# ohseokkwon/Foveated-Rendering-using-Ray-Tracing

Measured on AMD Instinct MI355X. Metric: Mrays/s + reconstructed fps @4K, 10% foveal density, 1/2/4/8 GPU, higher is better.
Workload: dtype f32

## Files before the change

foveated-rendering-using-ray-tracing_amd/csrc/ctx_buffers.cpp:

```cpp
#include <algorithm>
#include <array>

#include "ctx_internal.h"

using namespace fr;
using namespace fri;

namespace {
constexpr uint32_t kSnapMagic = 0x4E535246u;
constexpr uint32_t kSnapVersion = 1;
struct SnapHeader {
  uint32_t magic, version;
  int32_t width, height, pp_S, spp, scene, mask_mode;
  uint32_t accum, light_pending;
  float light_emission[3];
  int32_t diffuse_max_depth;
  float inv_vp[16], prev_vp[16], eye[3], prev_eye[3], gaze[2];
  uint64_t payload_bytes;
};
struct SnapPart {
  void* dev;
  size_t bytes;
};
std::array<SnapPart, 7> snap_parts(fr_ctx* c) {
// ... 168 lines not shown
  c->extra.settle(c);
  join_recon(c);
  hipSetDevice(c->cfg.device);
  const char* in = static_cast<const char*>(host);
  size_t off = sizeof(h);
  for (const SnapPart& p : snap_parts(c)) {
    HIP_TRY(c, hipMemcpyAsync(p.dev, in + off, p.bytes, hipMemcpyHostToDevice, c->stream));
    off += p.bytes;
  }
  HIP_TRY(c, hipStreamSynchronize(c->stream));
  c->accum = h.accum;
  c->light_pending = h.light_pending != 0;
  c->dsc.light_emission = mk3(h.light_emission[0], h.light_emission[1], h.light_emission[2]);
  c->U.diffuse_max_depth = h.diffuse_max_depth;
  c->U.mask_mode = h.mask_mode;
  memcpy(&c->U.inv_vp, h.inv_vp, sizeof(h.inv_vp));
  memcpy(&c->U.prev_vp, h.prev_vp, sizeof(h.prev_vp));
  memcpy(&c->U.eye, h.eye, sizeof(h.eye));
  memcpy(&c->U.prev_eye, h.prev_eye, sizeof(h.prev_eye));
  memcpy(&c->U.gaze, h.gaze, sizeof(h.gaze));
  c->lp_gaze = f2{-1e30f, -1e30f};
  c->lp_mode = -1;
  c->sib_prefix_fresh = false;
  c->hvalid_fresh = false;
  c->moved = false;
  return FR_OK;
}

}
```

foveated-rendering-using-ray-tracing_amd/csrc/ctx_create.cpp:

```cpp
#include <cmath>
#include <cstdlib>

#include "ctx_internal.h"

using namespace fr;
using fri::fail;

static thread_local std::string g_create_error;

int fri::fail(fr_ctx* c, int code, const std::string& msg) {
  if (c) c->err = msg; else g_create_error = msg;
  return code;
}

extern "C" {

const char* fr_version(void) { return "fovrt 0.2 (gfx950)"; }
int fr_abi_version(void) { return FOVRT_ABI_VERSION; }

int fr_config_default(fr_config* c) {
  if (!c) return FR_E_INVALID;
  memset(c, 0, sizeof(*c));
  c->abi_version = FOVRT_ABI_VERSION;
  c->width = 1024; c->height = 1024;
// ... 48 lines not shown
      return FR_TEX_F32;
    }
    out[i] = word;
  }
  return FR_TEX_RGBE;
}

static void read_env_knobs(fr_ctx* c) {
  if (const char* v = getenv("FOVRT_SHADE_CHUNK_REFR")) c->chunk_refr = (uint32_t)std::max(0, atoi(v));
  if (const char* v = getenv("FOVRT_SHADE_XCD_BANDS")) c->xcd_bands = atoi(v) != 0;
  if (const char* v = getenv("FOVRT_SHADE_HANDOFF")) c->handoff = (uint32_t)std::min(std::max(atoi(v), 0), 2);
  if (const char* v = getenv("FOVRT_TEX_PACKING")) c->tex_packing = atoi(v) != 0;
  if (const char* v = getenv("FOVRT_JFA_LAZY_OUTPUTS")) c->lazy_jfa_outputs = atoi(v) != 0;
  if (const char* v = getenv("FOVRT_EARLY_SETUP")) c->early_setup = atoi(v) != 0;
  if (const char* v = getenv("FOVRT_EXTRA_LAZY")) c->extra_lazy = atoi(v) != 0;
  if (const char* v = getenv("FOVRT_SIB_STRIP")) c->sib_strip = atoi(v) != 0;
  if (const char* v = getenv("FOVRT_SLOTS")) c->nslots = std::max(2, std::min(fr_ctx::MAX_SLOTS, atoi(v)));
  {
    const char* v = getenv("FOVRT_SHADE_BLOCKS_PER_CU");
    const int full = fr::shade_max_blocks_per_cu();
    c->shade_blocks_per_cu = v ? std::max(1, std::min(full, atoi(v))) : full;
  }
  if (const char* v = getenv("FOVRT_JFA_XCD")) c->jfa_xcd = atoi(v);
  if (const char* v = getenv("FOVRT_SIB_STRIP_MID")) c->sib_strip_mid = atoi(v);
  if (const char* v = getenv("FOVRT_ATROUS_ROWS2")) c->atrous_rows2 = atoi(v) != 0;
  if (const char* v = getenv("FOVRT_ATROUS_XCD")) c->atrous_xcd = atoi(v) != 0;
}

static std::vector<hipEvent_t*> timed_events(fr_ctx* c) {
  fr_ctx::StageEvents& t = c->tev;
  std::vector<hipEvent_t*> v = {&t.begin, &t.geometry, &t.sampling, &t.optimize, &t.shading, &t.end, &t.paths_begin,
                                &t.paths_end, &t.chain2_begin, &t.pullpush, &t.atrous, &t.chain1_begin, &t.jfa,
                                &t.sibson, &t.stage_begin, &t.stage_end, &c->ev_carry_fork, &c->ev_carry_done,
                                &c->ev_recon_fork, &c->ev_chain2_done, &c->ev_stream_join};
  for (auto& s : c->lat.ev)
    for (hipEvent_t* e : {&s.front_begin, &s.front_end, &s.jfa_end, &s.recon_end}) v.push_back(e);
  return v;
}

int fr_create(const fr_config* cfg_in, fr_ctx** out) {
  if (!out) return fail(nullptr, FR_E_INVALID, "out is NULL");
  *out = nullptr;
  fr_config cfg;
  if (cfg_in) cfg = *cfg_in; else fr_config_default(&cfg);
  if (cfg.abi_version != FOVRT_ABI_VERSION)
    return fail(nullptr, FR_E_INVALID, "fr_config.abi_version != FOVRT_ABI_VERSION (initialise it with fr_config_default)");
// ... 167 lines not shown
  const size_t atlas = (size_t)c->pp_S * (c->pp_S + c->pp_S / 2);
  if (compaction_tiles(c->W, c->H) > 1024) { c->err = "screen too large for the compaction scan"; return bail(FR_E_UNSUPPORTED); }
  for (int k = 0; k < c->nslots; k++)
    if (dalloc(&c->mask_p[k], N) != hipSuccess || dalloc(&c->ray_count_p[k], 4) != hipSuccess ||
        dalloc(&c->active_p[k], N) != hipSuccess) {
      c->err = "device allocation (work buffers) failed";
      return bail(FR_E_NOMEM);
    }
  c->mask = c->mask_p[0]; c->ray_count = c->ray_count_p[0]; c->active = c->active_p[0];
  for (int k = 0; k < fr_ctx::MAX_SLOTS; k++)
    if (dalloc(&c->owner_counts_p[k], FR_MAX_SHARD_RANKS) != hipSuccess) {
      c->err = "device allocation (work buffers) failed";
      return bail(FR_E_NOMEM);
    }
  if (dalloc(&c->bcount, nblocks) != hipSuccess ||
      hipHostMalloc((void**)&c->h_counts, sizeof(uint32_t) * fr_ctx::MAX_SLOTS * FR_MAX_SHARD_RANKS) != hipSuccess) {
    c->err = "allocation (shard counts) failed";
    return bail(FR_E_NOMEM);
  }
  memset(c->h_counts, 0, sizeof(uint32_t) * fr_ctx::MAX_SLOTS * FR_MAX_SHARD_RANKS);
  if (dalloc(&c->gclass, N) != hipSuccess || dalloc(&c->lp_cache, N) != hipSuccess ||
      dalloc(&c->lp_inv, logpolar_inv_words(c->W, c->H)) != hipSuccess || dalloc(&c->words, nwords) != hipSuccess ||
      dalloc(&c->counts, 4 * nblocks) != hipSuccess || dalloc(&c->offsets, 4 * nblocks) != hipSuccess ||
      dalloc(&c->tiles, 1024) != hipSuccess || dalloc(&c->jfa_a, N) != hipSuccess || dalloc(&c->jfa_b, N) != hipSuccess ||
      dalloc(&c->pull, atlas) != hipSuccess || dalloc(&c->push, atlas) != hipSuccess ||
      dalloc(&c->snap, pp_snap_count(c->pp_S)) != hipSuccess || dalloc(&c->stats, 1) != hipSuccess ||
      dalloc(&c->shade_ctr, shade_counter_words()) != hipSuccess || dalloc(&c->samples, std::max(N * cfg.spp, 2 * shade_fx_slots((uint32_t)N, cfg.spp, c->handoff, c->shade_blocks_per_cu))) != hipSuccess ||
      dalloc(&c->sample_help, std::max<size_t>(4 * shade_fx_slots((uint32_t)N, cfg.spp, c->handoff, c->shade_blocks_per_cu), 1)) != hipSuccess ||
      dalloc(&c->aux_p[0], N) != hipSuccess || dalloc(&c->aux_seed_p[0], N) != hipSuccess ||
      dalloc(&c->aux_p[1], N) != hipSuccess || dalloc(&c->aux_seed_p[1], N) != hipSuccess ||
      dalloc(&c->hvalid, N / 64 + 1) != hipSuccess ||
      hipMalloc((void**)&c->item_store, shade_item_store_f4(c->shade_blocks_per_cu) * sizeof(f4)) != hipSuccess ||
      (cfg.sibson_mode == 0 && (dalloc(&c->sib_prefix, (size_t)(c->W + 1) * c->H) != hipSuccess ||
                                dalloc(&c->sib_blocks, (size_t)sibson_prefix_blocks(c->W) * c->H) != hipSuccess ||
                                hipMalloc((void**)&c->sib_wide, ((size_t)c->W * c->H + 2) * sizeof(uint32_t)) != hipSuccess ||
                                hipMalloc((void**)&c->sib_strips, sibson_strip_words(c->W, c->H) * sizeof(uint32_t)) != hipSuccess ||
                                dalloc(&c->sib_rowp, sibson_rowp_texels(c->W, c->H)) != hipSuccess))) {
    c->err = "device allocation (work buffers) failed";
    return bail(FR_E_NOMEM);
  }
  c->aux = c->aux_p[0];
  c->aux_seed = c->aux_seed_p[0];
  {
    std::vector<float> ft((size_t)c->W + c->H);
    for (int x = 0; x < c->W; x++) ft[x] = ((float)x + 0.5f) / (float)c->W;
    for (int y = 0; y < c->H; y++) ft[(size_t)c->W + y] = ((float)y + 0.5f) / (float)c->H;
    if (!up(&c->ftab, ft)) { c->err = "device allocation (work buffers) failed"; return bail(FR_E_NOMEM); }
// ... 34 lines not shown
  const hipStream_t streams[5] = {c->stream, c->atrous_stream, c->sibson_stream, c->carry_stream, c->front_stream};
  for (hipStream_t s : streams) if (s) hipStreamSynchronize(s);
  auto fr = [](void* p) { if (p) hipFree(p); };
  fr(c->d_nodes); fr(c->d_tri); fr(c->d_prim); fr(c->d_shade); fr(c->d_pos);
  fr(c->spare_nodes); fr(c->spare_tri); fr(c->spare_prim); fr(c->spare_pos); fr(c->prev_pos); fr(c->shade_back);
  fr(c->pose_rest_pos); fr(c->pose_rest_nrm); fr(c->pose_stage_pos); fr(c->pose_stage_nrm);
  if (c->bvh_work) bvh_work_free(c->bvh_work);
  if (c->sah_work) sah_work_free(c->sah_work);
  if (c->nrm_work) normals_work_free(c->nrm_work);
  for (auto p : c->d_tex) fr(p);
  fr(c->d_mats); fr(c->d_texs);
  for (auto p : c->img) fr(p);
  for (int k = 0; k < fr_ctx::MAX_SLOTS; k++) { fr(c->mask_p[k]); fr(c->ray_count_p[k]); fr(c->active_p[k]); fr(c->owner_counts_p[k]); }
  fr(c->bcount); fr(c->shard_map); fr(c->front_need); fr(c->shade_radiance);
  if (c->h_counts) hipHostFree(c->h_counts);
  fr(c->geo);
  if (c->h_geo) hipHostFree(c->h_geo);
  fr(c->rb);
  if (c->h_rb) hipHostFree(c->h_rb);
  if (c->geo_read.ev) hipEventDestroy(c->geo_read.ev);
  for (auto& f : c->set_read) if (f.ev) hipEventDestroy(f.ev);
  if (c->update_done.ev) hipEventDestroy(c->update_done.ev);
  for (auto e : c->ev_counts) if (e) hipEventDestroy(e);
  fr(c->gclass); fr(c->lp_cache); fr(c->lp_inv); fr(c->words); fr(c->counts); fr(c->offsets); fr(c->tiles); fr(c->shade_ctr); fr(c->samples); fr(c->sample_help); fr(c->aux_p[0]); fr(c->aux_p[1]); fr(c->aux_seed_p[0]); fr(c->aux_seed_p[1]); fr(c->hvalid); fr(c->item_store); fr(c->jfa_a); fr(c->jfa_b); fr(c->ftab);
  fr(c->pull); fr(c->push); fr(c->snap); fr(c->stats); fr(c->sib_prefix); fr(c->sib_blocks); fr(c->sib_wide); fr(c->sib_strips); fr(c->sib_rowp);
  for (hipEvent_t* e : timed_events(c)) if (*e) hipEventDestroy(*e);
  if (c->front_done.ev) hipEventDestroy(c->front_done.ev);
  for (auto& f : c->trace_done) if (f.ev) hipEventDestroy(f.ev);
  for (auto& f : c->recon_done) if (f.ev) hipEventDestroy(f.ev);
  for (auto& f : c->jfa_done) if (f.ev) hipEventDestroy(f.ev);
  for (auto& q : c->kt_ev)
    for (auto e : q) if (e) hipEventDestroy(e);
  for (auto& q : c->fc_ev)
    for (auto e : q) if (e) hipEventDestroy(e);
  if (c->fc_ref) hipEventDestroy(c->fc_ref);
  for (hipStream_t s : streams) if (s) hipStreamDestroy(s);
  delete c;
  return FR_OK;
}

int fr_set_camera(fr_ctx* c, const fr_camera* cam) {
  if (!c || !cam) return FR_E_INVALID;
  FrameUniforms& U = c->U;
  memcpy(U.inv_vp.m, cam->inv_vp, sizeof(U.inv_vp.m));
  memcpy(U.prev_vp.m, cam->prev_vp, sizeof(U.prev_vp.m));
  U.eye = mk3(cam->eye[0], cam->eye[1], cam->eye[2]);
  U.prev_eye = mk3(cam->prev_eye[0], cam->prev_eye[1], cam->prev_eye[2]);
// ... 44 lines not shown
```

foveated-rendering-using-ray-tracing_amd/csrc/ctx_frame.cpp:

```cpp
#include <immintrin.h>
#include <sched.h>

#include <chrono>
#include <cmath>
#include <functional>

#include "ctx_internal.h"

using namespace fr;
using namespace fri;

namespace {
constexpr float kPollDeadlineMs = 10000.0f;
inline void cpu_relax() { _mm_pause(); }
hipError_t poll_event(hipEvent_t ev, float deadline_ms) {
  const auto t0 = std::chrono::steady_clock::now();
  for (uint32_t n = 1;; n++) {
    const hipError_t e = hipEventQuery(ev);
    if (e != hipErrorNotReady) return e;
    if ((n & 63u) == 0) {
      if (std::chrono::duration<float, std::milli>(std::chrono::steady_clock::now() - t0).count() > deadline_ms)
        return hipErrorNotReady;
      sched_yield();
    } else {
// ... 219 lines not shown
    case FR_BUF_DEPTH_CACHE: *phys = c->depth_cache; return FR_OK;
    case FR_BUF_DIFFUSE: *phys = P_DIFFUSE; return FR_OK;
    case FR_BUF_WEIGHT: *phys = P_wgt(c); return FR_OK;
    case FR_BUF_HISTORY: *phys = c->hist_cur; return FR_OK;
    case FR_BUF_HISTORY_CACHE: *phys = c->hist_cache; return FR_OK;
    case FR_BUF_SHADING: *phys = P_shd(c); return FR_OK;
    case FR_BUF_EXTRA: *phys = P_EXTRA; return FR_OK;
    case FR_BUF_JFA_COORD: *phys = P_JFA_COORD; return FR_OK;
    case FR_BUF_JFA_COLOR: *phys = P_JFA_COLOR; return FR_OK;
    case FR_BUF_SIBSON: *phys = P_SIBSON; return FR_OK;
    case FR_BUF_PULLPUSH: *phys = P_PULLPUSH; return FR_OK;
    case FR_BUF_ATROUS: *phys = c->atrous_out; return FR_OK;
    case FR_BUF_LOGPOLAR: *phys = P_LOGPOLAR; return FR_OK;
    case FR_BUF_LOGPOLAR_INVERSE: *phys = P_LOGPOLAR_INV; return FR_OK;
    default: return FR_E_INVALID;
  }
}

static int enqueue_jfa(fr_ctx* c, int in_buffer, hipStream_t stream = nullptr) {
  int p;
  if (resolve(c, in_buffer, &p)) return fail(c, FR_E_INVALID, "jfa: bad input buffer");
  const bool run_form = c->cfg.sibson_mode == 0;
  const bool lazy = run_form && c->lazy_jfa_outputs;
  c->jfa_final = launch_jfa(c->img[p], c->jfa_a, c->jfa_b, c->img[P_JFA_COORD], c->img[P_JFA_COLOR], c->ftab, c->W,
                            c->H, run_form ? c->sib_prefix : nullptr, run_form ? c->sib_blocks : nullptr, !lazy,
                            c->jfa_xcd, stream ? stream : c->stream);
  c->jfa_coord_owed = lazy;
  c->sib_prefix_fresh = run_form;
  return check_launch(c);
}
static int enqueue_sibson(fr_ctx* c, hipStream_t stream = nullptr) {
  if (c->cfg.sibson_mode == 1) {
    materialize_jfa(c, stream ? stream : c->stream);
    launch_sibson(c->img[P_JFA_COORD], c->img[P_JFA_COLOR], c->img[P_SIBSON], c->W, c->H, stream ? stream : c->stream);
  } else {
    launch_sibson_runs(c->img[P_JFA_COORD], c->jfa_final, c->img[P_JFA_COLOR], c->sib_prefix, c->sib_blocks, c->sib_rowp, c->sib_wide,
                       c->sib_strips, c->img[P_SIBSON], c->W, c->H, c->sib_prefix_fresh, c->sib_strip, c->sib_strip_mid,
                       c->jfa_coord_owed,
                       stream ? stream : c->stream);
  }
  return check_launch(c);
}
static int enqueue_pullpush(fr_ctx* c, int in_buffer, hipStream_t stream = nullptr) {
  int p;
  if (resolve(c, in_buffer, &p)) return fail(c, FR_E_INVALID, "pullpush: bad input buffer");
  launch_pullpush(c->img[p], c->pull, c->push, c->snap, c->img[P_PULLPUSH], c->W, c->H, stream ? stream : c->stream);
  return check_launch(c);
}
static int enqueue_atrous(fr_ctx* c, int count, int pos, int nrm, int col, hipStream_t stream = nullptr) {
  if (!stream) stream = c->stream;
  int pp, pn, pc;
  if (count < 1 || resolve(c, pos, &pp) || resolve(c, nrm, &pn) || resolve(c, col, &pc))
// ... 272 lines not shown
```

foveated-rendering-using-ray-tracing_amd/csrc/ctx_internal.h:

```cpp
#pragma once
#include <hip/hip_runtime.h>

#include <cstring>
#include <string>
#include <vector>

#include "../../include/fovrt.h"
#include "fr_device.h"
#include "k_launch.h"
#include "scene.h"

#define FR_MAX_SHARD_RANKS 64

using fr::f2;
using fr::f3;
using fr::u2;
using fr::f4;
using fr::BvhNode;
using fr::TriGeo;
using fr::TriShade;
using fr::DevMaterial;
using fr::DevTexture;
using fr::DevScene;
using fr::DevStats;
// ... 136 lines not shown
  uint8_t* lp_cache = nullptr;
  uint32_t* lp_inv = nullptr;
  f2 lp_gaze{-1e30f, -1e30f};
  int lp_mode = -1;
  unsigned long long* words = nullptr;
  uint32_t* counts = nullptr;
  uint32_t* offsets = nullptr;
  uint32_t* tiles = nullptr;
  uint32_t* ray_count = nullptr;
  uint32_t* active = nullptr;
  uint32_t* shade_ctr = nullptr;
  f4* samples = nullptr;
  unsigned long long* sample_help = nullptr;
  f4* item_store = nullptr;
  f4* aux = nullptr;
  uint32_t* aux_seed = nullptr;
  f4* aux_p[2] = {};
  uint32_t* aux_seed_p[2] = {};
  int aux_i = 0;
  unsigned long long* hvalid = nullptr;
  bool hvalid_fresh = false;
  bool setup_early = false;
  bool early_setup = true;
  u2 *jfa_a = nullptr, *jfa_b = nullptr;
  uint32_t chunk_refr = 0;
  uint32_t xcd_bands = 1;
  uint32_t handoff = 1;
  int shade_blocks_per_cu = 0;
  int jfa_xcd = 1;
  int sib_strip_mid = 0;
  bool atrous_rows2 = true;
  int atrous_xcd = 1;
  float* ftab = nullptr;
  f4 *pull = nullptr, *push = nullptr, *snap = nullptr;
  f4 *sib_prefix = nullptr, *sib_blocks = nullptr;
  uint32_t* sib_wide = nullptr;
  uint32_t* sib_strips = nullptr;
  f4* sib_rowp = nullptr;
  bool sib_prefix_fresh = false;
  const u2* jfa_final = nullptr;
  bool jfa_coord_owed = false;
  bool lazy_jfa_outputs = true;
  struct ExtraDebt {
    bool owed = false;
    FrameUniforms U;
    DevScene sc;
    const float* box = nullptr;
// ... 61 lines not shown
```

foveated-rendering-using-ray-tracing_amd/csrc/ctx_stats.cpp:

```cpp
#include <algorithm>
#include <cstdio>

#include "ctx_internal.h"

using namespace fr;
using namespace fri;

extern "C" {

int fr_get_stats(fr_ctx* c, fr_stats* s) {
  if (!c || !s) return FR_E_INVALID;
  DevStats d;
  HIP_TRY(c, hipMemcpyAsync(&d, c->stats, sizeof(d), hipMemcpyDeviceToHost, c->stream));
  HIP_TRY(c, hipStreamSynchronize(c->stream));
  s->gbuffer_primary = d.gbuffer_primary; s->primary = d.primary; s->shadow = d.shadow;
  s->diffuse_bounce = d.diffuse_bounce; s->mirror = d.mirror; s->refraction = d.refraction;
  s->reflection = d.reflection; s->truncated = d.truncated; s->overflow = d.bvh_overflow;
  for (int i = 0; i < 6; i++) s->diag[i] = d.pad[i];
  s->segments = d.gbuffer_primary + d.primary + d.shadow + d.diffuse_bounce + d.mirror + d.refraction + d.reflection;
  return FR_OK;
}

float fr__sqrt_le_bound(float s) { return sqrt_le_bound(s); }

int fr__sibson_counts(fr_ctx* c, uint32_t* out3) {
  if (!c || !out3 || !c->sib_strips) return FR_E_INVALID;
  hipSetDevice(c->cfg.device);
  HIP_TRY(c, hipDeviceSynchronize());
  HIP_TRY(c, hipMemcpy(out3, c->sib_strips, sizeof(uint32_t), hipMemcpyDeviceToHost));
  HIP_TRY(c, hipMemcpy(out3 + 1, c->sib_wide, 2 * sizeof(uint32_t), hipMemcpyDeviceToHost));
  return FR_OK;
}

int fr_kernel_timing(fr_ctx* c, int enable) {
  if (!c) return FR_E_INVALID;
  if (enable && !c->kt_ev[0][0])
    for (auto& q : c->kt_ev)
      for (auto& e : q) HIP_TRY(c, hipEventCreate(&e));
  c->kt_on = enable != 0;
  c->kt_next = c->kt_pending = 0;
  c->kt_frames = 0;
  c->kt_stage_ms = c->kt_kernel_ms = 0.0;
// ... 141 lines not shown
```

foveated-rendering-using-ray-tracing_amd/csrc/k_jfa.hip:

```cpp
#include <hip/hip_runtime.h>
#include <cmath>
#include "fr_device.h"
#include "k_launch.h"
#include "k_image.h"

namespace fr {


__global__ void k_jfa_init(const f4* __restrict__ in, u2* __restrict__ state, int W, int H, f2 screen) {
  const uint32_t N = (uint32_t)W * (uint32_t)H;
  for (uint32_t p = blockIdx.x * blockDim.x + threadIdx.x; p < N; p += gridDim.x * blockDim.x) {
    const float a = in[p].w;
    const uint32_t y = p / (uint32_t)W;
    const f2 uv = frag_uv(p - y * (uint32_t)W, y, screen);
    state[p] = a >= 1.0f ? u2{__float_as_uint(uv.x) | JFA_FLAG, __float_as_uint(uv.y) | JFA_FLAG}
                         : u2{JFA_UNSEEDED, __float_as_uint(uv.y)};
  }
}


typedef float jfa_v2 __attribute__((ext_vector_type(2)));
FR_DEV u2 jfa_pick(const u2 (&nb)[9], f2 me) {
  float d2[9];
  float dmin = INFINITY;
  const jfa_v2 m = {me.x, me.y};
#pragma unroll
  for (int i = 0; i < 9; i++) {
    const jfa_v2 c = {__uint_as_float(nb[i].x), __uint_as_float(nb[i].y)};
    const jfa_v2 dd = c + m;
    const jfa_v2 sq = dd * dd;
    d2[i] = sq.x + sq.y;
    dmin = fminf(dmin, d2[i]);
  }
  u2 r = nb[0];
  if (dmin != INFINITY) {
    const float bound = sqrt_le_bound(sqrtf(dmin));
#pragma unroll
    for (int i = 8; i >= 0; i--)
      if (d2[i] <= bound) r = nb[i];
// ... 18 lines not shown
  u2 r = nb[0];
  if (dmin != INFINITY) {
    const float bound = sqrt_le_bound(sqrtf(dmin));
    if (down) {
      if (d2[8] <= bound) r = nb[8];
      if (d2[7] <= bound) r = nb[7];
      if (d2[6] <= bound) r = nb[6];
    }
    if (d2[5] <= bound) r = nb[5];
    if (d2[4] <= bound) r = nb[4];
    if (up) {
      if (d2[3] <= bound) r = nb[3];
      if (d2[2] <= bound) r = nb[2];
      if (d2[1] <= bound) r = nb[1];
    }
    if (d2[0] <= bound) r = nb[0];
  }
  return r;
}


template <int JFA_ROWS>
__global__ __launch_bounds__(256) void k_jfa_step(const u2* __restrict__ src, u2* __restrict__ dst, int W, int H,
                                                  int step, const float* __restrict__ ftab, int xcd) {
  const uint32_t t = xcd ? xcd_tile(blockIdx.x, blockIdx.y, gridDim.x, gridDim.y) : blockIdx.y * gridDim.x + blockIdx.x;
  const int x = (int)(t % gridDim.x) * 64 + (threadIdx.x & 63);
  const int g = __builtin_amdgcn_readfirstlane((int)(t / gridDim.x) * 4 + (threadIdx.x >> 6));
  const int base = (g / step) * (JFA_ROWS * step) + g % step;
  if (x >= W || base >= H) return;
  const bool inl = x - step >= 0, inr = x + step < W;
  const int xl = inl ? x - step : x, xr = inr ? x + step : x;
  u2 L[JFA_ROWS + 2], C[JFA_ROWS + 2], R[JFA_ROWS + 2];
  bool in[JFA_ROWS + 2];
  const char* sb = reinterpret_cast<const char*>(src);
  auto ld = [&](uint32_t e) { return *reinterpret_cast<const u2*>(sb + e * 8u); };
#pragma unroll
  for (int m = 0; m < JFA_ROWS + 2; m++) {
    const int yr = base + (m - 1) * step;
    in[m] = yr >= 0 && yr < H;
    if (JFA_ROWS < 4 && !in[m]) {
      L[m] = C[m] = R[m] = u2{JFA_UNSEEDED, 0u};
      continue;
    }
    const uint32_t row = (uint32_t)(in[m] ? yr : base) * (uint32_t)W;
    L[m] = ld(row + (uint32_t)xl);
    C[m] = ld(row + (uint32_t)x);
    R[m] = ld(row + (uint32_t)xr);
    L[m].x = in[m] && inl ? L[m].x : JFA_UNSEEDED;
    C[m].x = in[m] ? C[m].x : JFA_UNSEEDED;
    R[m].x = in[m] && inr ? R[m].x : JFA_UNSEEDED;
  }
#pragma unroll
  for (int k = 0; k < JFA_ROWS; k++) {
    const int y = base + k * step;
    if (y < H) {
      const u2 nb[9] = {C[k + 1], L[k], C[k], R[k], L[k + 1], R[k + 1], L[k + 2], C[k + 2], R[k + 2]};
      *reinterpret_cast<u2*>(reinterpret_cast<char*>(dst) + ((uint32_t)y * (uint32_t)W + (uint32_t)x) * 8u) =
          JFA_ROWS < 4 ? jfa_pick_rows(nb, mk2(ftab[x], ftab[W + y]), in[k], in[k + 2])
                       : jfa_pick(nb, mk2(ftab[x], ftab[W + y]));
    }
  }
}

int jfa_rows(int H, int step) { return std::min(4, (H + step - 1) / step); }
int jfa_row_groups(int H, int step) {
  const int band = jfa_rows(H, step) * step;
  return ((H + band - 1) / band) * step;
}

__global__ void k_jfa_final(const u2* __restrict__ state, const f4* __restrict__ in, f4* __restrict__ coord,
                            f4* __restrict__ color, int W, int H, f2 screen) {
  const size_t N = (size_t)W * H;
  for (size_t p = blockIdx.x * (size_t)blockDim.x + threadIdx.x; p < N; p += (size_t)gridDim.x * blockDim.x) {
    const u2 s = state[p];
    const float sx = jfa_seeded(s.x) ? jfa_coord(s.x) : ((float)(p % (size_t)W) + 0.5f) / screen.x;
    const float sy = jfa_coord(s.y);
    const uint32_t ix = min((uint32_t)floorf(sx * screen.x), (uint32_t)W - 1);
    const uint32_t iy = min((uint32_t)floorf(sy * screen.y), (uint32_t)H - 1);
    const f4 c = in[(size_t)iy * W + ix];
    coord[p] = mk4(sx, sy, 0.0f, c.w);
    color[p] = c;
  }
}

template <bool OUT>
__global__ __launch_bounds__(64) void k_jfa_final_prefix(const u2* __restrict__ state, const f4* __restrict__ in,
                                                         f4* __restrict__ coord, f4* __restrict__ color,
                                                         f4* __restrict__ P, f4* __restrict__ T, int W, int H, int NB,
                                                         f2 screen) {
  const int lane = threadIdx.x;
  const int j = blockIdx.y, B = blockIdx.x;
  const int col = B * 64 + lane;
  f3 v = mk3(0.0f);
  if (col < W) {
    const size_t p = (size_t)j * W + col;
    const u2 s = state[p];
    const float sx = jfa_seeded(s.x) ? jfa_coord(s.x) : ((float)col + 0.5f) / screen.x;
    const float sy = jfa_coord(s.y);
    const uint32_t ix = min((uint32_t)floorf(sx * screen.x), (uint32_t)W - 1);
    const uint32_t iy = min((uint32_t)floorf(sy * screen.y), (uint32_t)H - 1);
    const f4 c = in[(size_t)iy * W + ix];
    if (OUT) coord[p] = mk4(sx, sy, 0.0f, c.w);
    color[p] = c;
    v = xyz(c);
  }
  f3 incl = v;
#pragma unroll
  for (int o = 1; o < 64; o <<= 1) {
    const float tx = __shfl_up(incl.x, o, 64), ty = __shfl_up(incl.y, o, 64), tz = __shfl_up(incl.z, o, 64);
    if (lane >= o) incl = incl + mk3(tx, ty, tz);
  }
  if (col <= W) P[(size_t)j * (W + 1) + col] = mk4(incl - v, 0.0f);
  if (lane == 63) T[(size_t)j * NB + B] = mk4(incl, 0.0f);
}

int jfa_max_step(int W, int H) {
  int m = 1;
  while (m * 2 < W || m * 2 < H) m *= 2;
  return m;
}

const u2* launch_jfa(const f4* in, u2* stateA, u2* stateB, f4* coord, f4* color, const float* ftab, int W, int H,
                     f4* sibP, f4* sibT, bool outputs, int xcd, hipStream_t stream) {
  const size_t N = (size_t)W * H;
  int blocks = (int)std::min<size_t>((N + 255) / 256, 8192);
  f2 screen = mk2((float)W, (float)H);
  hipLaunchKernelGGL(k_jfa_init, dim3(blocks), dim3(256), 0, stream, in, stateA, W, H, screen);
  u2* a = stateA;
  u2* b = stateB;
  for (int step = jfa_max_step(W, H); step >= 1; step /= 2) {
    dim3 grid((W + 63) / 64, (jfa_row_groups(H, step) + 3) / 4);
    auto k = jfa_rows(H, step) == 4 ? k_jfa_step<4> : jfa_rows(H, step) == 3 ? k_jfa_step<3>
           : jfa_rows(H, step) == 2 ? k_jfa_step<2> : k_jfa_step<1>;
    hipLaunchKernelGGL(k, grid, dim3(256), 0, stream, a, b, W, H, step, ftab, xcd);
    std::swap(a, b);
  }
  if (sibP) {
    const int NB = sibson_prefix_blocks(W);
    hipLaunchKernelGGL(outputs ? k_jfa_final_prefix<true> : k_jfa_final_prefix<false>, dim3(NB, H), dim3(64), 0, stream,
                       a, in, coord, color, sibP, sibT, W, H, NB, screen);
  } else {
    hipLaunchKernelGGL(k_jfa_final, dim3(blocks), dim3(256), 0, stream, a, in, coord, color, W, H, screen);
  }
  return a;
}

__global__ void k_jfa_coord(const u2* __restrict__ state, const f4* __restrict__ color, f4* __restrict__ coord, int W,
                            int H, f2 screen) {
  const size_t N = (size_t)W * H;
  for (size_t p = blockIdx.x * (size_t)blockDim.x + threadIdx.x; p < N; p += (size_t)gridDim.x * blockDim.x) {
    const u2 s = state[p];
    const float sx = jfa_seeded(s.x) ? jfa_coord(s.x) : ((float)(p % (size_t)W) + 0.5f) / screen.x;
    coord[p] = mk4(sx, jfa_coord(s.y), 0.0f, color[p].w);
  }
}
void launch_jfa_coord(const u2* state, const f4* color, f4* coord, int W, int H, hipStream_t stream) {
  const size_t N = (size_t)W * H;
  hipLaunchKernelGGL(k_jfa_coord, dim3((unsigned)std::min<size_t>((N + 255) / 256, 8192)), dim3(256), 0, stream, state,
                     color, coord, W, H, mk2((float)W, (float)H));
}

}
```

foveated-rendering-using-ray-tracing_amd/csrc/k_launch.h:

```cpp
#pragma once
#include <hip/hip_runtime.h>

#include <cstddef>
#include <cstdint>
#include <string>

#include "fr_device.h"

namespace fr {
void launch_gbuffer(const DevScene& sc, const FrameUniforms& U, f4* position, f4* normal, f4* depth, f4* diffuse,
                    f4* weight, uint8_t* gclass, DevStats* stats, const f3* cur_pos, const f3* prev_pos,
                    hipStream_t stream);
void launch_shade_paths(const DevScene& sc, const FrameUniforms& U, const uint32_t* active, const uint32_t* ray_count,
                        uint32_t max_active, const f4* weight, const f4* history_cache, uint32_t* chunk_ctr,
                        f4* samples, unsigned long long* help, DevStats* stats, f4* aux, uint32_t* aux_seed,
                        uint32_t chunk_refr, uint32_t xcd_bands, uint32_t handoff, int per_cu, f4* item_store,
                        hipStream_t stream);
int shade_max_blocks_per_cu();
size_t shade_item_store_f4(int per_cu);
void launch_sample_setup(const FrameUniforms& U, const uint32_t* active, const uint32_t* ray_count, uint32_t max_active,
                         const f4* weight, const f4* history_cache, const unsigned long long* hvalid, f4* aux,
                         uint32_t* aux_seed, hipStream_t stream);
void launch_shade_resolve(const FrameUniforms& U, const uint32_t* active, const uint32_t* ray_count,
                          uint32_t max_active, const f4* weight, const f4* history_cache, const f4* samples,
// ... 20 lines not shown
void diag_sample_trace(uint32_t* srec, uint32_t scap, uint32_t* wrec, uint32_t wcap, hipStream_t stream);
#endif

void launch_sampling(const FrameUniforms& U, const DevScene& sc, const f4* position, const f4* depth,
                     const f4* depth_cache, f4* weight, const f4* normal, const f4* diffuse, f4* extra, uint8_t* mask,
                     const uint8_t* gclass, unsigned long long* words, uint32_t* counts, int write_extra,
                     uint8_t* lp_cache, uint32_t* lp_inv, bool lp_refresh, uint32_t* bcount, bool motion,
                     const float* dev_box, hipStream_t stream);
void launch_extra(const FrameUniforms& U, const DevScene& sc, const f4* depth, const f4* weight, const f4* normal,
                  const f4* diffuse, f4* extra, const float* dev_box, hipStream_t stream);
size_t logpolar_inv_words(int W, int H);
void launch_owner_counts(const FrameUniforms& U, const uint32_t* bcount, uint32_t* owner_counts, hipStream_t stream);
void launch_mask_words(const uint8_t* mask, const uint8_t* gclass, int W, int H, unsigned long long* words,
                       uint32_t* counts, hipStream_t stream);
void launch_compaction(int W, int H, const unsigned long long* words, const uint32_t* counts, uint32_t* local_prefix,
                       uint32_t* tile_sum, uint32_t* ray_count, uint32_t* active, hipStream_t stream);
size_t compaction_tiles(int W, int H);

void launch_shard_pack(const FrameUniforms& U, const f4* buf, f4* slab, hipStream_t stream);
void launch_shard_unpack(const FrameUniforms& U, int rank, const f4* slab, f4* buf, hipStream_t stream);
void launch_logpolar(const f4* in, f4* fwd, f4* inv, int W, int H, f2 gaze, hipStream_t stream);
void launch_composite(const f4* views, int nviews, int W, int H, f4* out, hipStream_t stream);

const u2* launch_jfa(const f4* in, u2* stateA, u2* stateB, f4* coord, f4* color, const float* ftab, int W, int H,
                     f4* sibP, f4* sibT, bool outputs, int xcd, hipStream_t stream);
void launch_jfa_coord(const u2* state, const f4* color, f4* coord, int W, int H, hipStream_t stream);
void launch_sibson(const f4* coord, const f4* color, f4* out, int W, int H, hipStream_t stream);
void launch_sibson_runs(const f4* coord, const u2* state, const f4* color, f4* P, f4* T, f4* G, uint32_t* wide,
                        uint32_t* strips, f4* out, int W, int H, bool prefix_fresh, bool strip, int strip_mid,
                        bool coord_owed, hipStream_t stream);
int sibson_prefix_blocks(int W);
size_t sibson_strip_words(int W, int H);
size_t sibson_rowp_texels(int W, int H);

void launch_pullpush(const f4* in, f4* pull, f4* push, f4* snap, f4* out, int W, int H, hipStream_t stream);
bool launch_atrous(const f4* pos, const f4* nrm, const f4* col, f4* out, int W, int H, float c_phi, float n_phi,
                   float p_phi, float stepWidth, bool rows2, int xcd, hipStream_t stream);
int pp_size(int W, int H);
size_t pp_snap_count(int S);

struct BvhWork;
bool gpu_build_bvh(BvhWork** work, const f3* pos, int n, BvhNode* nodes, TriGeo* tri, int32_t* prim, int* num_nodes,
                   int* max_stack, int* depth, hipStream_t s, std::string& err);
void bvh_work_free(BvhWork* w);
bool bvh_work_prepare(BvhWork** w, int n, hipStream_t s, std::string& err);
bool bvh_builder_warm(BvhWork* w, hipStream_t s, std::string& err);
bool gpu_refit_bvh(BvhWork* work, const f3* pos, int n, BvhNode* nodes, int num_nodes, TriGeo* tri, const int32_t* prim,
                   hipStream_t s, std::string& err);
// ... 84 lines not shown
```

foveated-rendering-using-ray-tracing_amd/fovrt/__init__.py:

```python
from __future__ import annotations

import ctypes as C
import os
from dataclasses import dataclass

import numpy as np

_PKG_DIR = os.path.dirname(os.path.abspath(__file__))
LIB_PATH = os.path.join(os.path.dirname(_PKG_DIR), "libfovrt.so")
REPO_ROOT = os.path.dirname(os.path.dirname(_PKG_DIR))
DEFAULT_ASSET_DIR = os.path.join(REPO_ROOT, "assets")

ABI_VERSION = 2
GROUP_MAX_VIEW_RANKS = 16
FR_OK, FR_E_INVALID, FR_E_HIP, FR_E_NOMEM, FR_E_IO, FR_E_STATE, FR_E_UNSUPPORTED = 0, -1, -2, -3, -4, -5, -6
SCENE_BOX, SCENE_BUNNY, SCENE_VOKSELIA = 0, 1, 2
FR_BVH_REBUILD, FR_BVH_REFIT = 0, 1
FR_MEM_HOST, FR_MEM_DEVICE = 0, 1
FR_NORMALS_KEEP, FR_NORMALS_GIVEN, FR_NORMALS_RECOMPUTE = 0, 1, 2
MASK_SALIENCY, MASK_LOGPOLAR, MASK_UNIFORM2X2, MASK_ALL, MASK_LOGPOLAR_SIGNED = 0, 1, 2, 3, 4
PIPELINE_THROUGHPUT, PIPELINE_LATENCY = 0, 1
SCENES = {"box": SCENE_BOX, "bunny": SCENE_BUNNY, "vokselia": SCENE_VOKSELIA}
MASKS = {"saliency": MASK_SALIENCY, "logpolar": MASK_LOGPOLAR, "uniform": MASK_UNIFORM2X2, "all": MASK_ALL,
         "logpolar10": MASK_LOGPOLAR_SIGNED}
# ... 137 lines not shown
    "fr_set_geometry_overlap": [C.c_void_p, C.c_int],
    "fr_geometry_update_status": [C.c_void_p, C.POINTER(C.c_uint64), C.POINTER(C.c_uint64)],
    "fr_rebuild_bvh_enqueue": [C.c_void_p],
    "fr_bvh_rebuild_status": [C.c_void_p, C.POINTER(C.c_uint64), C.POINTER(C.c_uint64)],
    "fr_rebuild_bvh_enqueue_if": [C.c_void_p, C.c_float],
    "fr_set_rebuild_policy": [C.c_void_p, C.c_float, C.c_int],
    "fr_bvh_rebuild_policy_status": [C.c_void_p, C.POINTER(C.c_uint64), C.POINTER(C.c_uint64), C.POINTER(C.c_float),
                                     C.POINTER(C.c_float)],
    "fr_model_count": [C.c_void_p, C.POINTER(C.c_int)],
    "fr_model_info": [C.c_void_p, C.c_int, C.POINTER(C.c_char_p), C.POINTER(C.c_int), C.POINTER(C.c_int)],
    "fr_scene_model_count": [C.c_void_p, C.POINTER(C.c_int)],
    "fr_scene_model_info": [C.c_void_p, C.c_int, C.POINTER(C.c_char_p), C.POINTER(C.c_int), C.POINTER(C.c_int)],
    "fr_model_pose_enable": [C.c_void_p, C.c_int],
    "fr_set_model_transforms": [C.c_void_p, C.POINTER(C.c_float), C.c_size_t, C.c_int],
    "fr_set_model_transforms_enqueue": [C.c_void_p, C.POINTER(C.c_float), C.c_size_t],
    "fr_model_transforms": [C.c_void_p, C.POINTER(C.c_float), C.c_size_t],
    "fr_set_normals": [C.c_void_p, C.c_void_p, C.c_size_t, C.c_int],
    "fr_recompute_normals": [C.c_void_p, C.POINTER(C.c_float)],
    "fr_normal_groups": [C.c_void_p, C.POINTER(C.c_int32), C.c_size_t, C.POINTER(C.c_int)],
    "fr_set_motion_reprojection": [C.c_void_p, C.c_int],
    "fr_scene_normal_groups": [C.c_void_p, C.POINTER(C.c_int32), C.c_size_t, C.POINTER(C.c_int)],
    "fr_get_stats": [C.c_void_p, C.POINTER(fr_stats)],
    "fr_reset_stats": [C.c_void_p],
    "fr_kernel_timing": [C.c_void_p, C.c_int],
    "fr_kernel_times": [C.c_void_p, C.POINTER(fr_stage_times)],
    "fr_frame_clock": [C.c_void_p, C.c_int],
    "fr_frame_clock_read": [C.c_void_p, C.POINTER(C.c_float), C.POINTER(C.c_float), C.c_int, C.POINTER(C.c_int),
                            C.POINTER(C.c_int)],
    "fr_scene_export": [C.c_void_p, C.POINTER(fr_scene_arrays)],
    "fr_scene_create": [C.POINTER(fr_config), C.POINTER(C.c_void_p)],
    "fr_scene_get_arrays": [C.c_void_p, C.POINTER(fr_scene_arrays)],
    "fr_scene_destroy": [C.c_void_p],
    "fr_group_config_default": [C.POINTER(fr_group_config)],
    "fr_rccl_unique_id": [C.c_void_p],
    "fr_rccl_comm_init": [C.c_void_p, C.c_int, C.c_int, C.c_int, C.POINTER(C.c_void_p)],
    "fr_rccl_comm_destroy": [C.c_void_p],
    "fr_group_create": [C.POINTER(C.c_void_p), C.c_int, C.c_void_p, C.POINTER(fr_group_config), C.POINTER(C.c_void_p)],
    "fr_group_frame": [C.c_void_p, C.POINTER(fr_frame_timing)],
    "fr_group_composite": [C.c_void_p, C.c_void_p, C.c_size_t],
    "fr_group_rank_info": [C.c_void_p, C.c_int, C.POINTER(C.c_int), C.POINTER(C.c_int), C.POINTER(C.c_int),
                           C.POINTER(C.c_int)],
    "fr_group_tile_owners": [C.c_void_p, C.c_void_p, C.c_size_t],
    "fr_group_output_ranks": [C.c_void_p, C.c_int, C.POINTER(C.c_int), C.POINTER(C.c_int)],
    "fr_group_plan": [C.c_int, C.c_int, C.c_int, C.POINTER(fr_group_config), C.c_void_p, C.c_size_t],
    "fr_group_synchronize": [C.c_void_p],
    "fr_group_destroy": [C.c_void_p],
# ... 255 lines not shown

    def read(self, buf) -> np.ndarray:
        v = self.view(buf)
        if v.format == 0:
            out = np.empty((v.height, v.width, 4), np.float32)
        elif v.format == 1:
            out = np.empty((v.width,), np.uint32)
        else:
            out = np.empty((v.height, v.width), np.uint8)
        self._check(_lib.fr_read_buffer(self._ctx, int(buf), out.ctypes.data, out.nbytes))
        return out

    def write(self, buf, arr: np.ndarray):
        arr = np.ascontiguousarray(arr)
        self._check(_lib.fr_write_buffer(self._ctx, int(buf), arr.ctypes.data, arr.nbytes))

    def stats(self) -> dict:
        s = fr_stats()
        self._check(_lib.fr_get_stats(self._ctx, C.byref(s)))
        return {n: (list(getattr(s, n)) if n == "diag" else getattr(s, n)) for n, _ in fr_stats._fields_}

    def reset_stats(self):
        self._check(_lib.fr_reset_stats(self._ctx))

    def kernel_timing(self, enable: bool):
        self._check(_lib.fr_kernel_timing(self._ctx, 1 if enable else 0))

    def kernel_times(self) -> dict:
        t = fr_stage_times()
        self._check(_lib.fr_kernel_times(self._ctx, C.byref(t)))
        return {"frames": t.frames, "shading_ms": t.shading_ms, "shade_paths_ms": t.shade_paths_ms}

    def frame_clock(self, enable: bool):
        self._check(_lib.fr_frame_clock(self._ctx, 1 if enable else 0))

    def frame_clock_read(self, cap=100000):
        lat = (C.c_float * cap)()
        itv = (C.c_float * cap)()
        nl, ni = C.c_int(0), C.c_int(0)
        self._check(_lib.fr_frame_clock_read(self._ctx, lat, itv, cap, C.byref(nl), C.byref(ni)))
        return (np.frombuffer(lat, np.float32, nl.value).copy(), np.frombuffer(itv, np.float32, ni.value).copy())

    def _frame(self, fn, timing):
        t = fr_frame_timing() if timing else None
        self._check(fn(self._ctx, C.byref(t) if timing else None))
        if not timing:
# ... 529 lines not shown
```

include/fovrt.h:

```cpp
#ifndef FOVRT_H
#define FOVRT_H

#include <stddef.h>
#include <stdint.h>

#ifdef __cplusplus
extern "C" {
#endif

#define FOVRT_ABI_VERSION 2

typedef enum fr_status {
  FR_OK = 0,
  FR_E_INVALID = -1,
  FR_E_HIP = -2,
  FR_E_NOMEM = -3,
  FR_E_IO = -4,
  FR_E_STATE = -5,
  FR_E_UNSUPPORTED = -6
} fr_status;

typedef enum fr_scene_preset {
  FR_SCENE_BOX = 0,
  FR_SCENE_BUNNY = 1,
// ... 223 lines not shown
int fr_update_geometry_enqueue(fr_ctx* ctx, const void* xyz, const void* nrm, size_t ntris, int normals,
                               void* ready_event);
int fr_geometry_consumed(fr_ctx* ctx, void* stream);
int fr_set_geometry_overlap(fr_ctx* ctx, int on);
int fr_geometry_update_status(fr_ctx* ctx, uint64_t* applied, uint64_t* rejected);
#define FR_MAX_MODELS 16
int fr_model_count(fr_ctx* ctx, int* n);
int fr_model_info(fr_ctx* ctx, int i, const char** name, int* first_tri, int* ntris);
int fr_model_pose_enable(fr_ctx* ctx, int on);
int fr_set_model_transforms(fr_ctx* ctx, const float* m, size_t nmodels, int how);
int fr_set_model_transforms_enqueue(fr_ctx* ctx, const float* m, size_t nmodels);
int fr_model_transforms(fr_ctx* ctx, float* m, size_t nmodels);
int fr_set_motion_reprojection(fr_ctx* ctx, int on);
int fr_get_buffer(fr_ctx* ctx, int id, fr_buffer_view* view);
int fr_read_buffer(fr_ctx* ctx, int id, void* host, size_t bytes);
int fr_write_buffer(fr_ctx* ctx, int id, const void* host, size_t bytes);
int fr_copy_buffer(fr_ctx* ctx, int id, void* device_dst, size_t bytes);
int fr_snapshot_bytes(fr_ctx* ctx, size_t* bytes);
int fr_snapshot(fr_ctx* ctx, void* host, size_t bytes);
int fr_restore(fr_ctx* ctx, const void* host, size_t bytes);

int fr_get_stats(fr_ctx* ctx, fr_stats* stats);
int fr_reset_stats(fr_ctx* ctx);

typedef struct fr_stage_times {
  uint32_t frames;
  double shading_ms;
  double shade_paths_ms;
} fr_stage_times;
int fr_kernel_timing(fr_ctx* ctx, int enable);
int fr_kernel_times(fr_ctx* ctx, fr_stage_times* out);

int fr_frame_clock(fr_ctx* ctx, int enable);
int fr_frame_clock_read(fr_ctx* ctx, float* latency_ms, float* interval_ms, int cap, int* n_latency, int* n_interval);

typedef struct fr_scene_arrays {
  int num_tris;
  const float* pos;
  const float* nrm;
  const float* uv;
  const int32_t* flags;
  int num_materials;
  const int32_t* materials;
  int num_textures;
  const int32_t* tex_dims;
  const float* const* tex_data;
// ... 21 lines not shown
```

Baseline: 4912.

## Skip JFA flood steps when the seed mask is unchanged from the previous frame

The JFA init kernel now packs each frame's seed pattern into a per-wavefront bitmask with ballot and compares it against the stored mask from the previous frame. A generation-tagged control word records whether any word changed; when none did, every JFA step kernel returns early and the final kernels read a dedicated persistent result buffer F that still holds the previous flood result. This aims to remove the log-step JFA passes when the foveal sample pattern is static. In exchange it adds a bitmask read/write in init, a third state buffer, and force flags after restore or launch failure. It also exposes a skip counter through a new API.

```diff
diff --git a/foveated-rendering-using-ray-tracing_amd/csrc/ctx_buffers.cpp b/foveated-rendering-using-ray-tracing_amd/csrc/ctx_buffers.cpp
--- a/foveated-rendering-using-ray-tracing_amd/csrc/ctx_buffers.cpp
+++ b/foveated-rendering-using-ray-tracing_amd/csrc/ctx_buffers.cpp
@@ -214,6 +214,7 @@
   c->lp_gaze = f2{-1e30f, -1e30f};
   c->lp_mode = -1;
   c->sib_prefix_fresh = false;
+  c->jfa_force = true;
   c->hvalid_fresh = false;
   c->moved = false;
   return FR_OK;
diff --git a/foveated-rendering-using-ray-tracing_amd/csrc/ctx_create.cpp b/foveated-rendering-using-ray-tracing_amd/csrc/ctx_create.cpp
--- a/foveated-rendering-using-ray-tracing_amd/csrc/ctx_create.cpp
+++ b/foveated-rendering-using-ray-tracing_amd/csrc/ctx_create.cpp
@@ -94,6 +94,7 @@
     c->shade_blocks_per_cu = v ? std::max(1, std::min(full, atoi(v))) : full;
   }
   if (const char* v = getenv("FOVRT_JFA_XCD")) c->jfa_xcd = atoi(v);
+  if (const char* v = getenv("FOVRT_JFA_REUSE")) c->jfa_reuse = atoi(v) != 0;
   if (const char* v = getenv("FOVRT_SIB_STRIP_MID")) c->sib_strip_mid = atoi(v);
   if (const char* v = getenv("FOVRT_ATROUS_ROWS2")) c->atrous_rows2 = atoi(v) != 0;
   if (const char* v = getenv("FOVRT_ATROUS_XCD")) c->atrous_xcd = atoi(v) != 0;
@@ -307,7 +308,9 @@
   if (dalloc(&c->gclass, N) != hipSuccess || dalloc(&c->lp_cache, N) != hipSuccess ||
       dalloc(&c->lp_inv, logpolar_inv_words(c->W, c->H)) != hipSuccess || dalloc(&c->words, nwords) != hipSuccess ||
       dalloc(&c->counts, 4 * nblocks) != hipSuccess || dalloc(&c->offsets, 4 * nblocks) != hipSuccess ||
-      dalloc(&c->tiles, 1024) != hipSuccess || dalloc(&c->jfa_a, N) != hipSuccess || dalloc(&c->jfa_b, N) != hipSuccess ||
+      dalloc(&c->tiles, 1024) != hipSuccess || dalloc(&c->jfa.G, N) != hipSuccess || dalloc(&c->jfa.H, N) != hipSuccess ||
+      dalloc(&c->jfa.F, N) != hipSuccess || dalloc(&c->jfa.seeds, jfa_seed_words(c->W, c->H)) != hipSuccess ||
+      dalloc(&c->jfa.ctl, JFA_CTL_WORDS) != hipSuccess ||
       dalloc(&c->pull, atlas) != hipSuccess || dalloc(&c->push, atlas) != hipSuccess ||
       dalloc(&c->snap, pp_snap_count(c->pp_S)) != hipSuccess || dalloc(&c->stats, 1) != hipSuccess ||
       dalloc(&c->shade_ctr, shade_counter_words()) != hipSuccess || dalloc(&c->samples, std::max(N * cfg.spp, 2 * shade_fx_slots((uint32_t)N, cfg.spp, c->handoff, c->shade_blocks_per_cu))) != hipSuccess ||
@@ -388,7 +391,7 @@
   for (auto& f : c->set_read) if (f.ev) hipEventDestroy(f.ev);
   if (c->update_done.ev) hipEventDestroy(c->update_done.ev);
   for (auto e : c->ev_counts) if (e) hipEventDestroy(e);
-  fr(c->gclass); fr(c->lp_cache); fr(c->lp_inv); fr(c->words); fr(c->counts); fr(c->offsets); fr(c->tiles); fr(c->shade_ctr); fr(c->samples); fr(c->sample_help); fr(c->aux_p[0]); fr(c->aux_p[1]); fr(c->aux_seed_p[0]); fr(c->aux_seed_p[1]); fr(c->hvalid); fr(c->item_store); fr(c->jfa_a); fr(c->jfa_b); fr(c->ftab);
+  fr(c->gclass); fr(c->lp_cache); fr(c->lp_inv); fr(c->words); fr(c->counts); fr(c->offsets); fr(c->tiles); fr(c->shade_ctr); fr(c->samples); fr(c->sample_help); fr(c->aux_p[0]); fr(c->aux_p[1]); fr(c->aux_seed_p[0]); fr(c->aux_seed_p[1]); fr(c->hvalid); fr(c->item_store); fr(c->jfa.G); fr(c->jfa.H); fr(c->jfa.F); fr(c->jfa.seeds); fr(c->jfa.ctl); fr(c->ftab);
   fr(c->pull); fr(c->push); fr(c->snap); fr(c->stats); fr(c->sib_prefix); fr(c->sib_blocks); fr(c->sib_wide); fr(c->sib_strips); fr(c->sib_rowp);
   for (hipEvent_t* e : timed_events(c)) if (*e) hipEventDestroy(*e);
   if (c->front_done.ev) hipEventDestroy(c->front_done.ev);
diff --git a/foveated-rendering-using-ray-tracing_amd/csrc/ctx_frame.cpp b/foveated-rendering-using-ray-tracing_amd/csrc/ctx_frame.cpp
--- a/foveated-rendering-using-ray-tracing_amd/csrc/ctx_frame.cpp
+++ b/foveated-rendering-using-ray-tracing_amd/csrc/ctx_frame.cpp
@@ -265,12 +265,19 @@
   if (resolve(c, in_buffer, &p)) return fail(c, FR_E_INVALID, "jfa: bad input buffer");
   const bool run_form = c->cfg.sibson_mode == 0;
   const bool lazy = run_form && c->lazy_jfa_outputs;
-  c->jfa_final = launch_jfa(c->img[p], c->jfa_a, c->jfa_b, c->img[P_JFA_COORD], c->img[P_JFA_COLOR], c->ftab, c->W,
-                            c->H, run_form ? c->sib_prefix : nullptr, run_form ? c->sib_blocks : nullptr, !lazy,
-                            c->jfa_xcd, stream ? stream : c->stream);
+  if (!stream) stream = c->stream;
+  if (++c->jfa_gen == 0) {
+    hipMemsetAsync(c->jfa.ctl + JFA_CTL_CHANGED, 0, sizeof(uint32_t), stream);
+    c->jfa_gen = 1;
+  }
+  c->jfa_final = launch_jfa(c->img[p], c->jfa, c->jfa_gen, c->jfa_force || !c->jfa_reuse, c->img[P_JFA_COORD],
+                            c->img[P_JFA_COLOR], c->ftab, c->W, c->H, run_form ? c->sib_prefix : nullptr,
+                            run_form ? c->sib_blocks : nullptr, !lazy, c->jfa_xcd, stream);
   c->jfa_coord_owed = lazy;
   c->sib_prefix_fresh = run_form;
-  return check_launch(c);
+  const int rc = check_launch(c);
+  c->jfa_force = rc != FR_OK;
+  return rc;
 }
 static int enqueue_sibson(fr_ctx* c, hipStream_t stream = nullptr) {
   if (c->cfg.sibson_mode == 1) {
diff --git a/foveated-rendering-using-ray-tracing_amd/csrc/ctx_internal.h b/foveated-rendering-using-ray-tracing_amd/csrc/ctx_internal.h
--- a/foveated-rendering-using-ray-tracing_amd/csrc/ctx_internal.h
+++ b/foveated-rendering-using-ray-tracing_amd/csrc/ctx_internal.h
@@ -182,7 +182,10 @@
   bool hvalid_fresh = false;
   bool setup_early = false;
   bool early_setup = true;
-  u2 *jfa_a = nullptr, *jfa_b = nullptr;
+  fr::JfaState jfa = {};
+  uint32_t jfa_gen = 0;
+  bool jfa_force = true;
+  bool jfa_reuse = true;
   uint32_t chunk_refr = 0;
   uint32_t xcd_bands = 1;
   uint32_t handoff = 1;
diff --git a/foveated-rendering-using-ray-tracing_amd/csrc/ctx_stats.cpp b/foveated-rendering-using-ray-tracing_amd/csrc/ctx_stats.cpp
--- a/foveated-rendering-using-ray-tracing_amd/csrc/ctx_stats.cpp
+++ b/foveated-rendering-using-ray-tracing_amd/csrc/ctx_stats.cpp
@@ -18,6 +18,15 @@
   s->reflection = d.reflection; s->truncated = d.truncated; s->overflow = d.bvh_overflow;
   for (int i = 0; i < 6; i++) s->diag[i] = d.pad[i];
   s->segments = d.gbuffer_primary + d.primary + d.shadow + d.diffuse_bounce + d.mirror + d.refraction + d.reflection;
+  return FR_OK;
+}
+
+int fr_jfa_reuse_count(fr_ctx* c, uint32_t* skipped) {
+  if (!c || !skipped) return FR_E_INVALID;
+  join_recon(c);
+  hipSetDevice(c->cfg.device);
+  HIP_TRY(c, hipMemcpyAsync(skipped, c->jfa.ctl + JFA_CTL_SKIPPED, sizeof(uint32_t), hipMemcpyDeviceToHost, c->stream));
+  HIP_TRY(c, hipStreamSynchronize(c->stream));
   return FR_OK;
 }
 
diff --git a/foveated-rendering-using-ray-tracing_amd/csrc/k_jfa.hip b/foveated-rendering-using-ray-tracing_amd/csrc/k_jfa.hip
--- a/foveated-rendering-using-ray-tracing_amd/csrc/k_jfa.hip
+++ b/foveated-rendering-using-ray-tracing_amd/csrc/k_jfa.hip
@@ -7,14 +7,34 @@
 namespace fr {
 
 
-__global__ void k_jfa_init(const f4* __restrict__ in, u2* __restrict__ state, int W, int H, f2 screen) {
+__global__ __launch_bounds__(256) void k_jfa_init(const f4* __restrict__ in, u2* __restrict__ state,
+                                                  unsigned long long* __restrict__ seeds, uint32_t* ctl, uint32_t gen,
+                                                  int force, int W, int H, f2 screen) {
   const uint32_t N = (uint32_t)W * (uint32_t)H;
-  for (uint32_t p = blockIdx.x * blockDim.x + threadIdx.x; p < N; p += gridDim.x * blockDim.x) {
-    const float a = in[p].w;
-    const uint32_t y = p / (uint32_t)W;
-    const f2 uv = frag_uv(p - y * (uint32_t)W, y, screen);
-    state[p] = a >= 1.0f ? u2{__float_as_uint(uv.x) | JFA_FLAG, __float_as_uint(uv.y) | JFA_FLAG}
-                         : u2{JFA_UNSEEDED, __float_as_uint(uv.y)};
+  const uint32_t lane = threadIdx.x & 63u;
+  int changed = 0;
+  for (uint32_t p = blockIdx.x * blockDim.x + threadIdx.x; p - lane < N; p += gridDim.x * blockDim.x) {
+    bool seed = false;
+    if (p < N) {
+      const float a = in[p].w;
+      const uint32_t y = p / (uint32_t)W;
+      const f2 uv = frag_uv(p - y * (uint32_t)W, y, screen);
+      seed = a >= 1.0f;
+      state[p] = seed ? u2{__float_as_uint(uv.x) | JFA_FLAG, __float_as_uint(uv.y) | JFA_FLAG}
+                      : u2{JFA_UNSEEDED, __float_as_uint(uv.y)};
+    }
+    const unsigned long long bits = __ballot(seed);
+    if (lane == 0) {
+      const uint32_t w = p >> 6;
+      changed |= seeds[w] != bits;
+      seeds[w] = bits;
+    }
+  }
+  if (force) {
+    if (blockIdx.x == 0 && threadIdx.x == 0) atomicMax(&ctl[JFA_CTL_CHANGED], gen);
+  } else if (__syncthreads_or(changed) && threadIdx.x == 0 &&
+             __atomic_load_n(&ctl[JFA_CTL_CHANGED], __ATOMIC_RELAXED) != gen) {
+    atomicMax(&ctl[JFA_CTL_CHANGED], gen);
   }
 }
 
@@ -79,7 +99,9 @@
 
 template <int JFA_ROWS>
 __global__ __launch_bounds__(256) void k_jfa_step(const u2* __restrict__ src, u2* __restrict__ dst, int W, int H,
-                                                  int step, const float* __restrict__ ftab, int xcd) {
+                                                  int step, const float* __restrict__ ftab, int xcd,
+                                                  const uint32_t* __restrict__ ctl, uint32_t gen) {
+  if (ctl[JFA_CTL_CHANGED] != gen) return;
   const uint32_t t = xcd ? xcd_tile(blockIdx.x, blockIdx.y, gridDim.x, gridDim.y) : blockIdx.y * gridDim.x + blockIdx.x;
   const int x = (int)(t % gridDim.x) * 64 + (threadIdx.x & 63);
   const int g = __builtin_amdgcn_readfirstlane((int)(t / gridDim.x) * 4 + (threadIdx.x >> 6));
@@ -125,8 +147,14 @@
   return ((H + band - 1) / band) * step;
 }
 
+FR_DEV void jfa_count_skipped(uint32_t* ctl, uint32_t gen) {
+  if (blockIdx.x == 0 && blockIdx.y == 0 && threadIdx.x == 0 && ctl[JFA_CTL_CHANGED] != gen)
+    atomicAdd(&ctl[JFA_CTL_SKIPPED], 1u);
+}
+
 __global__ void k_jfa_final(const u2* __restrict__ state, const f4* __restrict__ in, f4* __restrict__ coord,
-                            f4* __restrict__ color, int W, int H, f2 screen) {
+                            f4* __restrict__ color, int W, int H, f2 screen, uint32_t* ctl, uint32_t gen) {
+  jfa_count_skipped(ctl, gen);
   const size_t N = (size_t)W * H;
   for (size_t p = blockIdx.x * (size_t)blockDim.x + threadIdx.x; p < N; p += (size_t)gridDim.x * blockDim.x) {
     const u2 s = state[p];
@@ -144,7 +172,8 @@
 __global__ __launch_bounds__(64) void k_jfa_final_prefix(const u2* __restrict__ state, const f4* __restrict__ in,
                                                          f4* __restrict__ coord, f4* __restrict__ color,
                                                          f4* __restrict__ P, f4* __restrict__ T, int W, int H, int NB,
-                                                         f2 screen) {
+                                                         f2 screen, uint32_t* ctl, uint32_t gen) {
+  jfa_count_skipped(ctl, gen);
   const int lane = threadIdx.x;
   const int j = blockIdx.y, B = blockIdx.x;
   const int col = B * 64 + lane;
@@ -177,29 +206,31 @@
   return m;
 }
 
-const u2* launch_jfa(const f4* in, u2* stateA, u2* stateB, f4* coord, f4* color, const float* ftab, int W, int H,
-                     f4* sibP, f4* sibT, bool outputs, int xcd, hipStream_t stream) {
+const u2* launch_jfa(const f4* in, const JfaState& st, uint32_t gen, bool force, f4* coord, f4* color,
+                     const float* ftab, int W, int H, f4* sibP, f4* sibT, bool outputs, int xcd, hipStream_t stream) {
   const size_t N = (size_t)W * H;
   int blocks = (int)std::min<size_t>((N + 255) / 256, 8192);
   f2 screen = mk2((float)W, (float)H);
-  hipLaunchKernelGGL(k_jfa_init, dim3(blocks), dim3(256), 0, stream, in, stateA, W, H, screen);
-  u2* a = stateA;
-  u2* b = stateB;
+  hipLaunchKernelGGL(k_jfa_init, dim3(blocks), dim3(256), 0, stream, in, st.G, st.seeds, st.ctl, gen, force ? 1 : 0, W,
+                     H, screen);
+  u2* a = st.G;
+  u2* b = st.H;
   for (int step = jfa_max_step(W, H); step >= 1; step /= 2) {
     dim3 grid((W + 63) / 64, (jfa_row_groups(H, step) + 3) / 4);
     auto k = jfa_rows(H, step) == 4 ? k_jfa_step<4> : jfa_rows(H, step) == 3 ? k_jfa_step<3>
            : jfa_rows(H, step) == 2 ? k_jfa_step<2> : k_jfa_step<1>;
-    hipLaunchKernelGGL(k, grid, dim3(256), 0, stream, a, b, W, H, step, ftab, xcd);
+    hipLaunchKernelGGL(k, grid, dim3(256), 0, stream, a, step == 1 ? st.F : b, W, H, step, ftab, xcd, st.ctl, gen);
     std::swap(a, b);
   }
   if (sibP) {
     const int NB = sibson_prefix_blocks(W);
     hipLaunchKernelGGL(outputs ? k_jfa_final_prefix<true> : k_jfa_final_prefix<false>, dim3(NB, H), dim3(64), 0, stream,
-                       a, in, coord, color, sibP, sibT, W, H, NB, screen);
+                       st.F, in, coord, color, sibP, sibT, W, H, NB, screen, st.ctl, gen);
   } else {
-    hipLaunchKernelGGL(k_jfa_final, dim3(blocks), dim3(256), 0, stream, a, in, coord, color, W, H, screen);
-  }
-  return a;
+    hipLaunchKernelGGL(k_jfa_final, dim3(blocks), dim3(256), 0, stream, st.F, in, coord, color, W, H, screen, st.ctl,
+                       gen);
+  }
+  return st.F;
 }
 
 __global__ void k_jfa_coord(const u2* __restrict__ state, const f4* __restrict__ color, f4* __restrict__ coord, int W,
diff --git a/foveated-rendering-using-ray-tracing_amd/csrc/k_launch.h b/foveated-rendering-using-ray-tracing_amd/csrc/k_launch.h
--- a/foveated-rendering-using-ray-tracing_amd/csrc/k_launch.h
+++ b/foveated-rendering-using-ray-tracing_amd/csrc/k_launch.h
@@ -66,8 +66,15 @@
 void launch_logpolar(const f4* in, f4* fwd, f4* inv, int W, int H, f2 gaze, hipStream_t stream);
 void launch_composite(const f4* views, int nviews, int W, int H, f4* out, hipStream_t stream);
 
-const u2* launch_jfa(const f4* in, u2* stateA, u2* stateB, f4* coord, f4* color, const float* ftab, int W, int H,
-                     f4* sibP, f4* sibT, bool outputs, int xcd, hipStream_t stream);
+struct JfaState {
+  u2 *G, *H, *F;
+  unsigned long long* seeds;
+  uint32_t* ctl;
+};
+enum { JFA_CTL_CHANGED = 0, JFA_CTL_SKIPPED = 1, JFA_CTL_WORDS = 2 };
+inline size_t jfa_seed_words(int W, int H) { return ((size_t)W * H + 63) / 64; }
+const u2* launch_jfa(const f4* in, const JfaState& st, uint32_t gen, bool force, f4* coord, f4* color,
+                     const float* ftab, int W, int H, f4* sibP, f4* sibT, bool outputs, int xcd, hipStream_t stream);
 void launch_jfa_coord(const u2* state, const f4* color, f4* coord, int W, int H, hipStream_t stream);
 void launch_sibson(const f4* coord, const f4* color, f4* out, int W, int H, hipStream_t stream);
 void launch_sibson_runs(const f4* coord, const u2* state, const f4* color, f4* P, f4* T, f4* G, uint32_t* wide,
diff --git a/foveated-rendering-using-ray-tracing_amd/fovrt/__init__.py b/foveated-rendering-using-ray-tracing_amd/fovrt/__init__.py
--- a/foveated-rendering-using-ray-tracing_amd/fovrt/__init__.py
+++ b/foveated-rendering-using-ray-tracing_amd/fovrt/__init__.py
@@ -183,6 +183,7 @@
     "fr_scene_normal_groups": [C.c_void_p, C.POINTER(C.c_int32), C.c_size_t, C.POINTER(C.c_int)],
     "fr_get_stats": [C.c_void_p, C.POINTER(fr_stats)],
     "fr_reset_stats": [C.c_void_p],
+    "fr_jfa_reuse_count": [C.c_void_p, C.POINTER(C.c_uint32)],
     "fr_kernel_timing": [C.c_void_p, C.c_int],
     "fr_kernel_times": [C.c_void_p, C.POINTER(fr_stage_times)],
     "fr_frame_clock": [C.c_void_p, C.c_int],
@@ -484,6 +485,11 @@
 
     def reset_stats(self):
         self._check(_lib.fr_reset_stats(self._ctx))
+
+    def jfa_reuse_count(self) -> int:
+        v = C.c_uint32()
+        self._check(_lib.fr_jfa_reuse_count(self._ctx, C.byref(v)))
+        return v.value
 
     def kernel_timing(self, enable: bool):
         self._check(_lib.fr_kernel_timing(self._ctx, 1 if enable else 0))
diff --git a/include/fovrt.h b/include/fovrt.h
--- a/include/fovrt.h
+++ b/include/fovrt.h
@@ -269,6 +269,7 @@
 
 int fr_get_stats(fr_ctx* ctx, fr_stats* stats);
 int fr_reset_stats(fr_ctx* ctx);
+int fr_jfa_reuse_count(fr_ctx* ctx, uint32_t* skipped);
 
 typedef struct fr_stage_times {
   uint32_t frames;
```

Result: faster. 5280 (median of 6 runs) (+7.5%).
